# yardenas/ethz-safe-learning

Hardware: AMD Instinct MI355X
Metric: planning steps/sec (CEM-MPC, N=2000 K=5 H=30) (higher is better)
Workload: dtype f32

## Files before the change

ethz_safe_learning_amd/_capi.py:

```python
from __future__ import annotations

import ctypes as C
import os

CEM_ABI_VERSION = 4
CEM_MAX_ACT = 32
CEM_MAX_COST_KINDS = 4
CEM_COMM_ID_BYTES = 128
CEM_MAX_BATCH = 256
CEM_TRAIN_MAX_BATCH = 4096
CEM_INIT_COLD, CEM_INIT_EXPLICIT, CEM_INIT_SHIFT = 0, 1, 2
CEM_VARIANT_CEM, CEM_VARIANT_SAFE, CEM_VARIANT_COST = 0, 1, 2
CEM_PARTICLES_MEAN, CEM_PARTICLES_LOWER_TAIL = 0, 1
CEM_CONSTRAINT_BETA, CEM_CONSTRAINT_BUDGET = 0, 1
CEM_REFIT_UNIFORM, CEM_REFIT_SOFTMAX = 0, 1
CEM_FORWARD_SPLIT, CEM_FORWARD_ALL = 0, 1

_HERE = os.path.dirname(os.path.abspath(__file__))
LIB_PATH = os.environ.get('CEM_MPC_LIB') or os.path.join(_HERE, 'lib', 'libcem_mpc_gfx950.so')

EXPORTED_SYMBOLS = [
    'cem_abi_version', 'cem_status_string', 'cem_last_hip_error', 'cem_weight_blob_floats',
    'cem_packed_weight_floats', 'cem_workspace_bytes', 'cem_pack_weights_host', 'cem_plan_tiles_host', 'cem_plan_segments_host', 'cem_rollout_residency',
    'cem_planner_create', 'cem_planner_destroy', 'cem_planner_layout', 'cem_planner_set_weights', 'cem_planner_set_weights_dev',
    'cem_planner_set_normaliser', 'cem_planner_plan', 'cem_plan_begin', 'cem_plan_rollout', 'cem_plan_select',
    'cem_plan_end', 'cem_comm_unique_id', 'cem_planner_comm_init', 'cem_planner_comm_destroy', 'cem_planner_comm_ranks', 'cem_plan_exchange', 'cem_planner_graph_status', 'cem_planner_launches_per_iteration', 'cem_unfold_sequences', 'cem_compute_objective', 'cem_scorer_reward', 'cem_scorer_cost', 'cem_fill_noise', 'cem_philox_words', 'cem_planner_set_timing', 'cem_planner_last_timing', 'cem_planner_last_timing_detail', 'cem_planner_select_mode', 'cem_planner_inject_fault',
    'cem_batch_workspace_bytes', 'cem_batch_planner_create', 'cem_planner_plan_batch', 'cem_planner_batch_capacity',
    'cem_planner_set_warm_start', 'cem_planner_set_initial_distribution', 'cem_planner_set_init_mode', 'cem_planner_reset_carry',
    'cem_planner_get_carry', 'cem_planner_set_carry_slots', 'cem_planner_set_particle_objective', 'cem_planner_get_particle_objective',
    'cem_planner_set_constraint', 'cem_planner_get_constraint', 'cem_planner_set_cost_budget', 'cem_planner_constraint_costs',
    'cem_planner_set_refit', 'cem_planner_get_refit', 'cem_planner_refit_stats',
    'cem_trainer_workspace_bytes', 'cem_trainer_blob_floats', 'cem_trainer_create', 'cem_trainer_destroy', 'cem_trainer_set_state',
    'cem_trainer_get_state', 'cem_trainer_weights_dev', 'cem_trainer_step', 'cem_trainer_steps', 'cem_trainer_eval', 'cem_trainer_forward',
]


class CemScorer(C.Structure):
    _fields_ = [
        ('goal_mode', C.c_int32), ('goal_lo', C.c_int32), ('goal_hi', C.c_int32),
        ('lidar_max_dist', C.c_float), ('goal_size', C.c_float), ('goal_reached_dist', C.c_float), ('reward_distance', C.c_float),
        ('reward_goal', C.c_float), ('reward_clip', C.c_float),
        ('constrain_indicator', C.c_int32), ('n_cost_kinds', C.c_int32),
        ('cost_lo', C.c_int32 * CEM_MAX_COST_KINDS), ('cost_hi', C.c_int32 * CEM_MAX_COST_KINDS),
        ('cost_size', C.c_float * CEM_MAX_COST_KINDS),
    ]


class CemConfig(C.Structure):
    _fields_ = [
# ... 61 lines not shown
    lib.cem_pack_weights_host.argtypes = [cfgp, vp, vp]
    lib.cem_plan_tiles_host.argtypes = [cfgp, i32p, i32p, vp, C.c_int32]
    lib.cem_plan_segments_host.argtypes = [cfgp, i32p, i32p]
    lib.cem_rollout_residency.argtypes = [C.c_int32, C.c_int32, i32p, i32p]
    lib.cem_planner_create.argtypes = [cfgp, vp, C.c_size_t, vp, C.POINTER(vp)]
    lib.cem_planner_destroy.argtypes = [vp]
    lib.cem_planner_layout.argtypes = [vp, C.POINTER(CemLayout)]
    lib.cem_planner_set_weights.argtypes = [vp, vp, C.c_size_t]
    lib.cem_planner_set_weights_dev.argtypes = [vp, vp, C.c_size_t]
    lib.cem_planner_set_normaliser.argtypes = [vp, vp, vp]
    lib.cem_planner_plan.argtypes = [vp, vp, C.c_uint64, C.c_uint64, vp, vp, vp, vp, fp, i32p]
    lib.cem_plan_begin.argtypes = [vp, vp, C.c_uint64, C.c_uint64, vp, vp]
    lib.cem_plan_rollout.argtypes = [vp, C.c_int32]
    lib.cem_plan_select.argtypes = [vp, C.c_int32]
    lib.cem_plan_end.argtypes = [vp, vp, vp, fp, i32p]
    lib.cem_unfold_sequences.argtypes = [vp, vp, vp, C.c_int32, C.c_int32, vp, C.c_uint64, C.c_uint64, vp, vp, vp]
    lib.cem_comm_unique_id.argtypes = [vp]
    lib.cem_planner_comm_init.argtypes = [vp, vp, C.c_int32, C.c_int32]
    lib.cem_planner_comm_destroy.argtypes = [vp]
    lib.cem_plan_exchange.argtypes = [vp]
    lib.cem_planner_graph_status.argtypes = [vp, i32p]
    lib.cem_planner_comm_ranks.argtypes = [vp, i32p]
    lib.cem_planner_launches_per_iteration.argtypes = [vp, i32p]
    lib.cem_compute_objective.argtypes = [vp, vp, C.c_int32, C.c_int32, vp]
    lib.cem_scorer_reward.argtypes = [vp, vp, vp, C.c_int32, vp, vp]
    lib.cem_scorer_cost.argtypes = [vp, vp, C.c_int32, vp]
    lib.cem_fill_noise.argtypes = [vp, C.c_uint64, C.c_uint64, vp, vp, vp]
    lib.cem_philox_words.argtypes = [vp, C.c_uint64, C.c_uint64] + [C.c_uint32] * 6 + [vp]
    lib.cem_planner_select_mode.argtypes = [vp, i32p]
    lib.cem_planner_inject_fault.argtypes = [vp, C.c_int32]
    lib.cem_planner_set_timing.argtypes = [vp, C.c_int32]
    lib.cem_planner_last_timing.argtypes = [vp, fp, i32p, fp]
    lib.cem_planner_last_timing_detail.argtypes = [vp, fp, fp]
    lib.cem_batch_workspace_bytes.restype = C.c_size_t
    lib.cem_batch_workspace_bytes.argtypes = [cfgp, C.c_int32]
    lib.cem_batch_planner_create.argtypes = [cfgp, C.c_int32, vp, C.c_size_t, vp, C.POINTER(vp)]
    lib.cem_planner_plan_batch.argtypes = [vp, C.c_int32, vp, C.c_uint64, vp, vp, vp, vp, vp, vp, vp]
    lib.cem_planner_batch_capacity.argtypes = [vp, i32p]
    lib.cem_planner_set_warm_start.argtypes = [vp, C.POINTER(CemWarmStart)]
    lib.cem_planner_set_initial_distribution.argtypes = [vp, C.c_int32, vp, vp]
    lib.cem_planner_set_init_mode.argtypes = [vp, C.c_int32, C.c_int32]
    lib.cem_planner_reset_carry.argtypes = [vp, C.c_int32]
    lib.cem_planner_get_carry.argtypes = [vp, C.c_int32, vp, vp, i32p]
    lib.cem_planner_set_carry_slots.argtypes = [vp, C.c_int32, vp]
    lib.cem_planner_set_particle_objective.argtypes = [vp, C.c_int32, C.c_int32]
    lib.cem_planner_get_particle_objective.argtypes = [vp, i32p, i32p]
# ... 35 lines not shown
```

ethz_safe_learning_amd/csrc/cem_capi.hip:

```cpp
#include "cem_device.h"
#include "cem_score.h"
#include "cem_refit_weighted.h"
#include "cem_train.h"
#include "cem_train_tile.h"
#include "cem_forward.h"
#include "cem_rollout_split.h"
#include "cem_rollout_wide.h"
#include "cem_pack.h"
#include "../../include/cem_mpc.h"

#include <dlfcn.h>
#include <link.h>

#include <algorithm>
#include <atomic>
#include <chrono>
#include <cmath>
#include <cstdio>
#include <cstdlib>
#include <cstring>
#include <limits>
#include <mutex>
#include <new>
#include <string>
// ... 560 lines not shown
        dl_iterate_phdr(count_hip_runtimes, &libs);
        if (libs.size() > 1) {
            std::fprintf(stderr, "cem_mpc: %zu HIP runtimes are loaded in this process:", libs.size());
            for (const auto &l : libs) std::fprintf(stderr, " %s", l.c_str());
            std::fprintf(stderr, "\ncem_mpc: device memory and streams of one are foreign to the other — load libcem_mpc_gfx950.so AFTER the runtime that owns them (INTEGRATION.md)\n");
        }
    });
}
}

struct cem_planner {
    cem_config_t cfg;
    Dims d;
    Layout lay;
    char *ws;
    hipStream_t stream;
    bool own_stream;
    int rc;
    int n_tiles;
    int n_seg, seg_len, n_pinned;
    bool have_weights;
    bool in_plan;
    bool sample_in_rollout;
    const float *eps_act, *eps_model;
    CtrlBlock *h_ctrl;
    float *h_result;
    WarmCtl *h_warm; const WarmCtl *d_h_warm;
    uint32_t plan_seq;
    const CtrlBlock *d_h_ctrl; float *d_h_result;
    bool timing; std::vector<hipEvent_t> ev; float roll_ms, sel_ms, red_ms, samp_ms; int roll_n;
    std::vector<std::pair<int, int>> ev_kind;
    hipGraph_t graph; hipGraphExec_t gexec; bool graph_ready;
    ScorerDev sc;
    ScorerDev sc_roll;
    float alpha, beta;
    void *comm;
    int plans_since_comm;
    bool graph_failed;
    size_t sel_dyn_limit;
    int fused_resident;
    bool sel_zeroed;
    bool fuse_banned;
    bool inject_capture_fail;
    uint32_t inject_next;
    char *scratch; size_t scratch_bytes;
    std::vector<float> h_etab;
// ... 135 lines not shown
int cem_plan_segments_host(const cem_config_t *cfg, int32_t *segments_out, int32_t *steps_per_segment_out)
{
    int st = validate(cfg); if (st) return st;
    const Dims d = make_dims(cfg);
    const Plan pl = make_plan(cfg, d);
    if (segments_out) *segments_out = pl.n_seg;
    if (steps_per_segment_out) *steps_per_segment_out = pl.seg_len;
    return CEM_OK;
}

int cem_rollout_residency(int32_t chunks_per_tile, int32_t input_blocks_per_wave, int32_t *table_out, int32_t *runtime_out)
{
    if (chunks_per_tile < 1 || chunks_per_tile > 4 || input_blocks_per_wave < 1 || input_blocks_per_wave > 2) return CEM_ERR_INVALID_ARG;
    for (int seg = 0; seg < 2; ++seg) {
        if (table_out) table_out[seg] = kResidentStatic[seg][input_blocks_per_wave - 1][chunks_per_tile - 1];
        if (runtime_out)
            runtime_out[seg] = with_tile_shape(chunks_per_tile, input_blocks_per_wave, 0, [&](auto R, auto F) { return query_resident<R(), F()>(seg != 0); });
    }
    return CEM_OK;
}

}

static int planner_create(const cem_config_t *cfg, int32_t mb, void *workspace, size_t workspace_bytes, void *hip_stream, cem_planner_t **out)
{
    int st = mb ? validate_batch(cfg, mb) : validate(cfg); if (st) return st;
    if (!workspace || !out) return CEM_ERR_INVALID_ARG;
    warn_if_two_hip_runtimes();
    cem_planner *h = new (std::nothrow) cem_planner();
    if (!h) return CEM_ERR_INVALID_ARG;
    h->cfg = *cfg; h->d = make_dims(cfg);
    h->batch = mb; h->n_states = warm_slots(h);
    const size_t nb = (size_t)warm_slots(h);
    h->lay = make_layout(cfg, h->d, max_tiles_of(h->d), mb);
    if (workspace_bytes < h->lay.total || ((uintptr_t)workspace & 255)) { delete h; return CEM_ERR_WORKSPACE; }
    h->ws = (char *)workspace; h->stream = (hipStream_t)hip_stream; h->own_stream = false;
    if (!h->stream) {
        if (hipStreamCreateWithFlags(&h->stream, hipStreamNonBlocking) != hipSuccess) { g_last_hip = (int)hipGetLastError(); delete h; return CEM_ERR_HIP; }
        h->own_stream = true;
    }
    { const Plan pl = make_plan(cfg, h->d, mb); h->rc = pl.rc; h->n_seg = pl.n_seg; h->seg_len = pl.seg_len; h->n_pinned = pl.n_pinned;
      const int slots = real_cus() * ((h->d.wide || h->d.split) ? 1 : resident_workgroups(h->d.NFW, pl.rc, pl.n_seg > 1));
      h->sample_in_rollout = (long long)nb * pl.n_tiles <= slots;
      if (const char *e = std::getenv("CEM_FORCE_SAMPLER"))
          h->sample_in_rollout = std::strcmp(e, "kernel") != 0; }
    h->have_weights = false; h->in_plan = false; h->eps_act = h->eps_model = nullptr;
    h->timing = false; h->roll_ms = h->sel_ms = h->red_ms = h->samp_ms = 0.f; h->roll_n = 0;
    h->graph = nullptr; h->gexec = nullptr; h->graph_ready = false; h->tail_m = 0;
    h->cost_m = 0; h->budget_dev = nullptr; h->cstat_obj = nullptr; h->cstat_obj_n = 0; h->last_cstat = nullptr; h->last_cstat_n = h->last_cstat_problems = 0;
    h->refit_kind = CEM_REFIT_UNIFORM; h->refit_tau = 0.f; h->refit_beta = 0.f; h->refit_dev = nullptr; h->refit_ran = false;
    h->h_budget.assign(nb, std::numeric_limits<float>::infinity());
    h->comm = nullptr; h->plans_since_comm = 0; h->graph_failed = false;
    h->h_ctrl = nullptr; h->h_result = nullptr; h->h_warm = nullptr; h->d_h_warm = nullptr; h->pack_desc = nullptr; h->n_pack_desc = 0;
    h->warm = cem_warm_start_t{}; h->warm.shift = 1; h->warm_staged = 0; h->warm_save_skipped = false;
    h->slot_mode.assign(nb, CEM_INIT_COLD); h->carry_valid.assign(nb, 0); h->have_expl.assign(nb, 0); h->carry_at.assign(nb, -1);
    h->slot_of.resize(nb); for (size_t b = 0; b < nb; ++b) h->slot_of[b] = (int32_t)b;
    h->h_expl.assign(nb * 2 * h->d.H * h->d.A, 0.f);
    h->scratch = nullptr; h->scratch_bytes = 0; h->sel_zeroed = false; h->plan_seq = 0; h->fuse_banned = false; h->inject_next = 0; h->inject_capture_fail = false;
    auto fail = [&](int status) { g_last_hip = (int)hipGetLastError(); release_handle(h); return status; };
    const size_t result_bytes = mb ? nb * CEM_RESULT_WORDS * 4 : 64 * 4;
    if (hipHostMalloc((void **)&h->h_ctrl, nb * sizeof(CtrlBlock), hipHostMallocMapped | hipHostMallocCoherent) != hipSuccess ||
        hipHostMalloc((void **)&h->h_result, result_bytes, hipHostMallocMapped | hipHostMallocCoherent) != hipSuccess ||
        hipHostMalloc((void **)&h->h_warm, sizeof(WarmCtl) + nb * sizeof(WarmProb), hipHostMallocMapped | hipHostMallocCoherent) != hipSuccess) return fail(CEM_ERR_HIP);
    {
        const std::vector<PackDesc> table = build_pack_table(h->d);
        h->n_pack_desc = (uint32_t)table.size();
        const size_t image_bytes = h->d.wide ? wide_image_floats(h->d) * 4 : (size_t)h->d.member_stride_f4 * 16 - 4096;
        if (table.size() * (h->d.split ? 3072 : 1024) != image_bytes) return fail(CEM_ERR_STATE);
// ... 389 lines not shown
    const Dims &d = h->d; const Layout &l = h->lay; char *ws = h->ws;
    const bool queued = h->n_seg > 1 && !h->eps_model;
    RolloutParams rp; fill_rollout_common(h, rp);
    rp.tiles = (const TileDesc *)(ws + l.tiles); rp.s0 = nullptr; rp.actions = (const float *)(ws + l.actions);
    rp.eps_model = h->eps_model ? h->eps_model + (size_t)it * d.H * d.Btot * d.O : nullptr;
    const bool cost_obj = h->cfg.variant == CEM_VARIANT_COST;
    rp.ret = (float *)(ws + l.returns); rp.costs = h->cfg.variant != CEM_VARIANT_CEM ? (uint8_t *)(ws + l.costs) : nullptr;
    rp.H = d.H; rp.Bloc = d.Bloc; rp.Btot = d.Btot; rp.it = it; rp.variant = cost_obj ? (int)CEM_VARIANT_SAFE : h->cfg.variant; rp.check_done = 1;
    rp.stamps = (long long *)(ws + l.stamps);
    rp.musig = (const float *)(ws + l.musig); rp.eps_act = h->eps_act ? h->eps_act + (size_t)it * d.N * d.H * d.A : nullptr;
    rp.act_bounds = (const float *)(ws + l.act_bounds); rp.actions_w = (float *)(ws + l.actions); rp.act_pad_w = (float *)(ws + l.act_pad);
    rp.pad_shift = d.O - 4 * d.act_q0; rp.pad_floats = 4 * d.act_nq; rp.N = d.N; rp.Nloc = d.Nloc; rp.n_off = d.n_off; rp.n_tiles = h->n_tiles;
    const int nb = warm_slots(h);
    rp.tiles_per_problem = h->batch ? h->n_tiles : 0;
    rp.eps_act_pstride = (long long)d.I * d.N * d.H * d.A; rp.eps_model_pstride = (long long)d.I * d.H * d.Btot * d.O;
    if (!h->sample_in_rollout) {
        const int total = d.N * d.H * ((d.A + 3) / 4);
        TimedLaunch timed(h, 3);
        hipLaunchKernelGGL(cem_sample_kernel, dim3(std::min((total + 255) / 256, 2048), nb), dim3(256), 0, h->stream, rp);
        HIPCHK(hipGetLastError());
        rp.musig = nullptr;
    }
    TimedLaunch timed(h, 0);
    if (d.wide) HIPCHK(launch_rollout_wide(h, rp, h->n_tiles, rp.eps_model ? 1 : 0));
    else if (d.split) HIPCHK(launch_rollout_split(h->rc, d.NFW, rp.eps_model ? 1 : 0, rp, h->n_tiles, h->stream));
    else if (rp.eps_model) HIPCHK(launch_rollout<1>(h->rc, d.NFW, rp, nb * h->n_tiles, h->stream));
    else if (queued) {
        rp.seg_queue = (uint32_t *)(ws + l.seg_queue); rp.seg_flags = (uint32_t *)(ws + l.seg_flags); rp.seg_state = (f4 *)(ws + l.seg_state);
        rp.seg_len = h->seg_len; rp.n_seg = h->n_seg; rp.n_pinned = h->n_pinned;
        HIPCHK(launch_rollout_seg(h->rc, d.NFW, rp, h->n_pinned + h->n_seg * (h->n_tiles - h->n_pinned), h->stream));
    } else HIPCHK(launch_rollout<0>(h->rc, d.NFW, rp, nb * h->n_tiles, h->stream));
    timed.stop();
    if (fold_reduce) return CEM_OK;

    const ReduceParams sp = fill_score(h, rp.ret, rp.costs, (float *)(ws + l.scores_local), h->cost_m ? h->budget_dev + nb : nullptr, d.Nloc, d.H, 1, true);
    h->sel_zeroed = true;
    if (h->cost_m) note_plan_cstat(h);
    TimedLaunch timed_reduce(h, 2);
    HIPCHK(launch_score(h, sp, nb));
    return CEM_OK;
}

bool folds_reduce(const cem_planner *h)
{
    const Dims &d = h->d;
    if (d.W != 1 || h->comm || h->cfg.variant != CEM_VARIANT_CEM) return false;
    if (h->tail_m) return false;
// ... 635 lines not shown
    return CEM_OK;
}

int cem_planner_comm_destroy(cem_planner_t *h)
{
    if (!h) return CEM_ERR_INVALID_ARG;
    if (h->in_plan) return CEM_ERR_STATE;
    if (h->comm) {
        HIPCHK(hipStreamSynchronize(h->stream));
        if (Rccl *r = rccl()) r->CommDestroy(h->comm);
        h->comm = nullptr;
        drop_graph(h);
    }
    return CEM_OK;
}

int cem_planner_graph_status(const cem_planner_t *h, int32_t *status_out)
{
    if (!h || !status_out) return CEM_ERR_INVALID_ARG;
    *status_out = h->graph_ready ? 1 : (h->graph_failed ? 2 : 0);
    return CEM_OK;
}

int cem_planner_launches_per_iteration(const cem_planner_t *h, int32_t *launches_out)
{
    if (!h || !launches_out) return CEM_ERR_INVALID_ARG;
    const int mode = select_mode_now(h);
    *launches_out = 1 + (h->sample_in_rollout ? 0 : 1) + (folds_reduce(h) ? 0 : 1) + (mode == 2 ? 8 : (mode == 3 ? 2 : 1)) +
                    (h->refit_kind == CEM_REFIT_SOFTMAX ? 1 : 0);
    return CEM_OK;
}

int cem_plan_exchange(cem_planner_t *h)
{
    if (!h) return CEM_ERR_INVALID_ARG;
    if (!h->in_plan || !h->comm) return CEM_ERR_STATE;
    return enqueue_exchange(h);
}

static int ensure_scratch(cem_planner *h, size_t bytes)
{
    if (bytes <= h->scratch_bytes) return CEM_OK;
    if (h->scratch) { HIPCHK(hipStreamSynchronize(h->stream)); HIPCHK(hipFree(h->scratch)); h->scratch = nullptr; h->scratch_bytes = 0; }
    const size_t want = align256(bytes + bytes / 2);
    HIPCHK(hipMalloc((void **)&h->scratch, want));
    h->scratch_bytes = want;
// ... 459 lines not shown
```

ethz_safe_learning_amd/csrc/cem_device.h:

```cpp
#pragma once
#include <hip/hip_runtime.h>
#include <stdint.h>

typedef float f4 __attribute__((ext_vector_type(4)));

#define CEM_U 128
#define CEM_ET_NMIN 0
#define CEM_ET_RDELTA 1
#define CEM_ET_BMU 2
#define CEM_ET_BVAR 3
#define CEM_ET_OBS 4
#define CEM_ET_ACT 5
#define CEM_ET_SEL0 6
#define CEM_ET_SEL1 7
#define CEM_ET_ROWS 8
#define CEM_NG 8
#define CEM_NKIND 5
#define CEM_PART_FLOATS (CEM_NKIND * 4 * 64)
#define CEM_TAB_LDS_BYTES (CEM_ET_ROWS * CEM_U * 4)
#define CEM_ROLLOUT_LDS_BYTES(RC_) ((size_t)2 * (RC_) * CEM_NG * 1024 + CEM_PART_FLOATS * 4 + CEM_TAB_LDS_BYTES)

struct TileDesc {
    int32_t row_base;
    int32_t cnt;
// ... 361 lines not shown
    if (!p.musig) return;
    const TileDesc td = p.tiles[tile_idx];
    const bool natural = natural_all || td.row_base < p.Nloc;
    const int AZ = (p.A + 3) >> 2, nst = t1 - t0;
    const PhiloxKey key = cem_key(p.ctrl + b);
    const int own = td.cnt * nst * AZ;
    for (int idx = (int)threadIdx.x; idx < own; idx += 256) {
        const int z = idx % AZ, tt = (idx / AZ) % nst, r_ = idx / (AZ * nst);
        cem_sample_store(p, td.act_base + r_, t0 + tt, z, key, true, natural, b);
    }
    if (foreign && p.Nloc < p.N) {
        const long long total = (long long)(p.N - p.Nloc) * p.H * AZ;
        const long long per = (total + p.n_tiles - 1) / p.n_tiles;
        const long long lo = per * tile_idx, hi = (lo + per < total) ? lo + per : total;
        for (long long idx = lo + (long long)threadIdx.x; idx < hi; idx += 256) {
            const int z = (int)(idx % AZ), t = (int)((idx / AZ) % p.H);
            const int jn = (int)(idx / ((long long)AZ * p.H));
            cem_sample_store(p, jn < p.n_off ? jn : jn + p.Nloc, t, z, key, false);
        }
    }
    if (WAIT) cem_tile_sample_join();
}

__global__ __launch_bounds__(256) void cem_sample_kernel(const RolloutParams p)
{
    const int b = (int)blockIdx.y;
    if (p.check_done && p.ctrl[b].done) return;
    const int AZ = (p.A + 3) >> 2;
    const int total = p.N * p.H * AZ;
    const PhiloxKey key = cem_key(p.ctrl + b);
    for (int idx = blockIdx.x * blockDim.x + threadIdx.x; idx < total; idx += gridDim.x * blockDim.x) {
        const int z = idx % AZ, t = (idx / AZ) % p.H, n = idx / (AZ * p.H);
        cem_sample_store(p, n, t, z, key, true, true, b);
    }
}

#include "cem_rollout_common.h"

#define CEM_TAB(TABL_, ROW_, TV_) (*reinterpret_cast<const f4 *>((TABL_) + (ROW_) * 512 + (TV_)))
#define CEM_SEL0_LDS(TABL_, TV_) CEM_TAB(TABL_, CEM_ET_SEL0, TV_)

template <int RC, int NFW, int MODE, bool SEG>
__device__ __forceinline__ void cem_rollout_tile(const RolloutParams &p, char *smem, const int tile_idx, const int t_begin, const int t_end, const int b = 0)
{
    const int tid = (int)((threadIdx.x + 64u * (unsigned)((tile_idx + (tile_idx >> 8)) & 3)) & 255u);
    const int w = __builtin_amdgcn_readfirstlane(tid >> 6);
    const int lane = tid & 63;
    const int j = lane & 15, q = lane >> 4;
    const TileDesc td = p.tiles[tile_idx];
    const bool resumed = SEG && t_begin > 0;
    const int wbk = 0;
    const __amdgpu_buffer_rsrc_t seg_rs = __builtin_amdgcn_make_buffer_rsrc(
        SEG ? const_cast<f4 *>(p.seg_state + (size_t)(tile_idx - p.n_pinned) * (2 * NFW * RC * 256 + 64)) : const_cast<f4 *>(p.wpack), 0,
        (2 * NFW * RC * 256 + 64) * 16, 0x00020000);
    const int O = p.O, A = p.A, H = p.H;
    constexpr int XB = RC * CEM_NG * 1024;
    constexpr int LA = CEM_LDS_AHEAD_OF(RC, NFW);
    float *part = reinterpret_cast<float *>(smem + 2 * XB);
// ... 297 lines not shown
    const int tile = (int)(item >> 8), seg = (int)(item & 255u);
    const int t0 = seg * p.seg_len, t1 = (t0 + p.seg_len < p.H) ? t0 + p.seg_len : p.H;
    cem_tile_sample_actions<false>(p, tile, t0, t1 < p.H ? t1 + 1 : p.H, seg == 0, false);
    cem_rollout_tile<RC, NFW, 0, true>(p, smem, tile, t0, t1);
    if (t1 == p.H) {
        if (threadIdx.x == 0) item_s = atomicAdd(p.seg_queue + 2, 1u);
        __syncthreads();
        if (item_s == n_float - 1u) {
            const int n_ready = (int)n_float * (p.n_seg - 1);
            for (int i = (int)threadIdx.x; i < n_ready; i += 256) __hip_atomic_store(p.seg_flags + i, 0u, __ATOMIC_RELAXED, __HIP_MEMORY_SCOPE_AGENT);
            if (threadIdx.x < 3) __hip_atomic_store(p.seg_queue + threadIdx.x, 0u, __ATOMIC_RELAXED, __HIP_MEMORY_SCOPE_AGENT);
        }
    }
    if (t1 < p.H) {
        __builtin_amdgcn_s_waitcnt(0x0F70);
        __syncthreads();
        if (threadIdx.x == 0) {
            const uint32_t pos = atomicAdd(p.seg_queue + 1, 1u);
            __hip_atomic_store(p.seg_flags + pos, (((uint32_t)tile << 8) | (uint32_t)(seg + 1)) + 1u, __ATOMIC_RELAXED, __HIP_MEMORY_SCOPE_AGENT);
        }
    }
}

struct WarmProb {
    int32_t mode;
    int32_t slot;
    int32_t save_slot;
    int32_t pad;
};
struct WarmCtl { int32_t shift, tail, sigma_rule, two_phase ; float sigma_floor[32]; WarmProb prob[1];  };
#define CEM_WARM_LDS_PROBS 256

struct InitParams { CtrlBlock *ctrl; const CtrlBlock *host_ctrl; float *musig; int32_t HA, A; float mu0[32], sigma0[32]; uint32_t *seg_queue, *seg_flags; int32_t n_ready;
                    int32_t n_prob;
                    const WarmCtl *warm;
                    float *carry;
                    const float *expl;      };

__global__ void cem_init_kernel(const InitParams p)
{
    const int i = blockIdx.x * blockDim.x + threadIdx.x;
    const int np = p.n_prob > 1 ? p.n_prob : 1;
    WarmProb wp0{}; float fl0 = 0.f; int32_t hd0 = 0;
    if (blockIdx.x == 0) {
        if ((int)threadIdx.x < np) wp0 = p.warm->prob[threadIdx.x];
        if (threadIdx.x < 32) fl0 = p.warm->sigma_floor[threadIdx.x];
// ... 1186 lines not shown
    if (p.eps_act) {
        const int AZ = (p.A + 3) >> 2;
        const size_t total = (size_t)p.I * p.N * p.H * AZ;
        for (size_t idx = gid; idx < total; idx += gsz) {
            const int z = idx % AZ, t = (idx / AZ) % p.H, n = (idx / ((size_t)AZ * p.H)) % p.N, it = idx / ((size_t)AZ * p.H * p.N);
            const f4 e = cem_normal4((uint32_t)n, (uint32_t)t, (uint32_t)it, (uint32_t)z, CEM_STREAM_ACT, cem_key(p.ctrl));
            for (int r = 0; r < 4; ++r) if (4 * z + r < p.A) p.eps_act[(((size_t)it * p.N + n) * p.H + t) * p.A + 4 * z + r] = e[r];
        }
    }
    if (p.eps_model) {
        const int OZ = (p.O + 3) >> 2;
        const size_t total = (size_t)p.I * p.H * p.B * OZ;
        for (size_t idx = gid; idx < total; idx += gsz) {
            const int fq = idx % OZ; const size_t row = (idx / OZ) % p.B; const int t = (idx / ((size_t)OZ * p.B)) % p.H, it = idx / ((size_t)OZ * p.B * p.H);
            const f4 e = cem_normal4((uint32_t)row, (uint32_t)t, (uint32_t)it, (uint32_t)fq, CEM_STREAM_MODEL, cem_key(p.ctrl));
            for (int r = 0; r < 4; ++r) if (4 * fq + r < p.O) p.eps_model[(((size_t)it * p.H + t) * p.B + row) * p.O + 4 * fq + r] = e[r];
        }
    }
    if (p.eps_out && gid < (size_t)p.A) {
        const f4 e = cem_normal4((uint32_t)(gid >> 2), 0u, 0u, 0u, CEM_STREAM_OUT, cem_key(p.ctrl));
        p.eps_out[gid] = e[gid & 3];
    }
}
```

ethz_safe_learning_amd/planner.py:

```python
from __future__ import annotations

import ctypes as C
import math
from dataclasses import dataclass, field
from typing import List, Optional, Sequence, Tuple

import numpy as np

from . import _capi


@dataclass
class ScorerConfig:
    goal_slice: Tuple[int, int]
    observe_goal_lidar: bool = True
    lidar_max_dist: float = 4.0
    goal_size: float = 0.3
    reward_distance: float = 1.0
    reward_goal: float = 1.0
    reward_clip: float = 10.0
    constrain_indicator: bool = True
    cost_kinds: List[Tuple[int, int, float]] = field(default_factory=list)


# ... 320 lines not shown
        with self._torch.cuda.device(self.device):
            _capi.check(self.lib.cem_planner_comm_init(self.h, buf, c.world_size, c.rank), 'cem_planner_comm_init')
        self.has_comm = True

    def comm_ranks(self):
        n = C.c_int32()
        _capi.check(self.lib.cem_planner_comm_ranks(self.h, C.byref(n)), 'cem_planner_comm_ranks')
        return n.value

    def comm_destroy(self):
        _capi.check(self.lib.cem_planner_comm_destroy(self.h), 'cem_planner_comm_destroy')
        self.has_comm = False

    def graph_status(self):
        st = C.c_int32()
        _capi.check(self.lib.cem_planner_graph_status(self.h, C.byref(st)), 'cem_planner_graph_status')
        return ('eager', 'graph', 'graph-unsupported')[st.value]

    def launches_per_iteration(self):
        n = C.c_int32()
        _capi.check(self.lib.cem_planner_launches_per_iteration(self.h, C.byref(n)), 'cem_planner_launches_per_iteration')
        return n.value

    def set_particle_objective(self, kind='mean', m=0):
        if kind not in PARTICLE_OBJECTIVES:
            raise ValueError("kind is 'mean' or 'lower_tail'")
        _capi.check(self.lib.cem_planner_set_particle_objective(self.h, PARTICLE_OBJECTIVES[kind], int(m)), 'cem_planner_set_particle_objective')

    def particle_objective(self):
        kind, m = C.c_int32(), C.c_int32()
        _capi.check(self.lib.cem_planner_get_particle_objective(self.h, C.byref(kind), C.byref(m)), 'cem_planner_get_particle_objective')
        return ('mean', 'lower_tail')[kind.value], m.value

    def set_constraint(self, kind='beta', worst_cost_particles=0):
        if kind not in CONSTRAINTS:
            raise ValueError("kind is 'beta' or 'budget'")
        _capi.check(self.lib.cem_planner_set_constraint(self.h, CONSTRAINTS[kind], int(worst_cost_particles)), 'cem_planner_set_constraint')

    def constraint(self):
        kind, m = C.c_int32(), C.c_int32()
        _capi.check(self.lib.cem_planner_get_constraint(self.h, C.byref(kind), C.byref(m)), 'cem_planner_get_constraint')
        return ('beta', 'budget')[kind.value], m.value

    def set_cost_budget(self, budget):
        b = np.ascontiguousarray(np.asarray(budget, np.float32).reshape(-1))
        self.budget_staged = None
# ... 424 lines not shown
```

include/cem_mpc.h:

```cpp
#ifndef CEM_MPC_H
#define CEM_MPC_H

#include <stddef.h>
#include <stdint.h>

#ifdef __cplusplus
extern "C" {
#endif

#define CEM_ABI_VERSION 4
#define CEM_MAX_ACT 32
#define CEM_MAX_COST_KINDS 4
#define CEM_MAX_BATCH 256

enum cem_status {
    CEM_OK = 0,
    CEM_ERR_INVALID_ARG = 1,
    CEM_ERR_UNSUPPORTED = 2,
    CEM_ERR_SPLIT = 3,
    CEM_ERR_WORKSPACE = 4,
    CEM_ERR_HIP = 5,
    CEM_ERR_NO_WEIGHTS = 6,
    CEM_ERR_STATE = 7,
    CEM_ERR_COMM = 8,
// ... 94 lines not shown
int cem_planner_set_normaliser(cem_planner_t *h, const float *inputs_min, const float *inputs_max );
int cem_planner_set_weights_dev(cem_planner_t *h, const float *blob_dev, size_t n_floats);

int cem_planner_plan(cem_planner_t *h, const float *state, uint64_t seed, uint64_t call,
                     const float *eps_act_dev, const float *eps_model_dev, const float *eps_out_host,
                     float *action_out, float *best_score_out, int32_t *iters_out);

int cem_plan_begin(cem_planner_t *h, const float *state, uint64_t seed, uint64_t call,
                   const float *eps_act_dev, const float *eps_model_dev);
int cem_plan_rollout(cem_planner_t *h, int32_t it);
int cem_plan_select(cem_planner_t *h, int32_t it);
int cem_plan_end(cem_planner_t *h, const float *eps_out_host, float *action_out, float *best_score_out, int32_t *iters_out);

#define CEM_COMM_ID_BYTES 128
int cem_comm_unique_id(void *id_out );
int cem_planner_comm_init(cem_planner_t *h, const void *id , int32_t n_ranks, int32_t rank);
int cem_planner_comm_destroy(cem_planner_t *h);
int cem_planner_comm_ranks(const cem_planner_t *h, int32_t *n_ranks_out);
int cem_plan_exchange(cem_planner_t *h);
int cem_planner_select_mode(const cem_planner_t *h, int32_t *mode_out);
int cem_planner_inject_fault(cem_planner_t *h, int32_t kind);
int cem_planner_graph_status(const cem_planner_t *h, int32_t *status_out);
int cem_planner_launches_per_iteration(const cem_planner_t *h, int32_t *launches_out);

int cem_unfold_sequences(cem_planner_t *h, const float *s0_dev, const float *actions_dev, int32_t n_rows, int32_t horizon,
                         const float *eps_model_dev, uint64_t seed, uint64_t call,
                         float *traj_out_dev, float *mu_out_dev, float *sd_out_dev);

int cem_compute_objective(cem_planner_t *h, const float *traj_dev, int32_t n_rows, int32_t horizon, float *scores_out_dev);

int cem_scorer_reward(cem_planner_t *h, const float *obs_dev, const float *next_obs_dev, int32_t n, float *reward_out_dev,
                      uint8_t *goal_achieved_out_dev);
int cem_scorer_cost(cem_planner_t *h, const float *obs_dev, int32_t n, float *cost_out_dev);

int cem_fill_noise(cem_planner_t *h, uint64_t seed, uint64_t call, float *eps_act_dev, float *eps_model_dev, float *eps_out_dev);

int cem_philox_words(cem_planner_t *h, uint64_t seed, uint64_t call, uint32_t stream, uint32_t iteration, uint32_t t, uint32_t sub,
                     uint32_t idx0, uint32_t n, uint32_t *words_out_dev);

int cem_planner_set_timing(cem_planner_t *h, int32_t enable);
int cem_planner_last_timing(cem_planner_t *h, float *rollout_ms_total, int32_t *rollout_launches, float *select_ms_total);
int cem_planner_last_timing_detail(cem_planner_t *h, float *reduce_ms_total, float *sampler_ms_total);

size_t cem_batch_workspace_bytes(const cem_config_t *cfg, int32_t max_batch);
int cem_batch_planner_create(const cem_config_t *cfg, int32_t max_batch, void *workspace, size_t workspace_bytes, void *hip_stream,
                             cem_planner_t **out);
// ... 78 lines not shown
```

Baseline: 528.9.

## Add specialized lean rollout kernel for single-member, four-layer, RC=1 configurations

Adds a dedicated rollout kernel specialized for RC=1, NFW=1, four hidden layers and in-rollout sampling. It stages the action mean/sigma and bounds in LDS, computes clipped actions inline, and buffers kept actions in LDS so they are written out once at the end instead of per step. It also rotates wave priorities per step. The host picks this path automatically when eligible and keeps the generic path behind an environment override. The trade-off is extra LDS use and a second kernel to maintain. The weak symbol means the generic path is used if the new object is not linked.

```diff
diff --git a/ethz_safe_learning_amd/_capi.py b/ethz_safe_learning_amd/_capi.py
--- a/ethz_safe_learning_amd/_capi.py
+++ b/ethz_safe_learning_amd/_capi.py
@@ -24,7 +24,7 @@
     'cem_packed_weight_floats', 'cem_workspace_bytes', 'cem_pack_weights_host', 'cem_plan_tiles_host', 'cem_plan_segments_host', 'cem_rollout_residency',
     'cem_planner_create', 'cem_planner_destroy', 'cem_planner_layout', 'cem_planner_set_weights', 'cem_planner_set_weights_dev',
     'cem_planner_set_normaliser', 'cem_planner_plan', 'cem_plan_begin', 'cem_plan_rollout', 'cem_plan_select',
-    'cem_plan_end', 'cem_comm_unique_id', 'cem_planner_comm_init', 'cem_planner_comm_destroy', 'cem_planner_comm_ranks', 'cem_plan_exchange', 'cem_planner_graph_status', 'cem_planner_launches_per_iteration', 'cem_unfold_sequences', 'cem_compute_objective', 'cem_scorer_reward', 'cem_scorer_cost', 'cem_fill_noise', 'cem_philox_words', 'cem_planner_set_timing', 'cem_planner_last_timing', 'cem_planner_last_timing_detail', 'cem_planner_select_mode', 'cem_planner_inject_fault',
+    'cem_plan_end', 'cem_comm_unique_id', 'cem_planner_comm_init', 'cem_planner_comm_destroy', 'cem_planner_comm_ranks', 'cem_plan_exchange', 'cem_planner_graph_status', 'cem_planner_launches_per_iteration', 'cem_planner_rollout_path', 'cem_unfold_sequences', 'cem_compute_objective', 'cem_scorer_reward', 'cem_scorer_cost', 'cem_fill_noise', 'cem_philox_words', 'cem_planner_set_timing', 'cem_planner_last_timing', 'cem_planner_last_timing_detail', 'cem_planner_select_mode', 'cem_planner_inject_fault',
     'cem_batch_workspace_bytes', 'cem_batch_planner_create', 'cem_planner_plan_batch', 'cem_planner_batch_capacity',
     'cem_planner_set_warm_start', 'cem_planner_set_initial_distribution', 'cem_planner_set_init_mode', 'cem_planner_reset_carry',
     'cem_planner_get_carry', 'cem_planner_set_carry_slots', 'cem_planner_set_particle_objective', 'cem_planner_get_particle_objective',
@@ -132,6 +132,7 @@
     lib.cem_planner_graph_status.argtypes = [vp, i32p]
     lib.cem_planner_comm_ranks.argtypes = [vp, i32p]
     lib.cem_planner_launches_per_iteration.argtypes = [vp, i32p]
+    lib.cem_planner_rollout_path.argtypes = [vp, i32p]
     lib.cem_compute_objective.argtypes = [vp, vp, C.c_int32, C.c_int32, vp]
     lib.cem_scorer_reward.argtypes = [vp, vp, vp, C.c_int32, vp, vp]
     lib.cem_scorer_cost.argtypes = [vp, vp, C.c_int32, vp]
diff --git a/ethz_safe_learning_amd/csrc/cem_capi.hip b/ethz_safe_learning_amd/csrc/cem_capi.hip
--- a/ethz_safe_learning_amd/csrc/cem_capi.hip
+++ b/ethz_safe_learning_amd/csrc/cem_capi.hip
@@ -1,4 +1,5 @@
 #include "cem_device.h"
+#include "cem_rollout_lean.h"
 #include "cem_score.h"
 #include "cem_refit_weighted.h"
 #include "cem_train.h"
@@ -606,6 +607,7 @@
     bool have_weights;
     bool in_plan;
     bool sample_in_rollout;
+    bool lean_rollout;
     const float *eps_act, *eps_model;
     CtrlBlock *h_ctrl;
     float *h_result;
@@ -787,6 +789,13 @@
 
 }
 
+static bool lean_eligible(const cem_planner *h, int rc)
+{
+    const Dims &d = h->d;
+    return launch_rollout_lean != nullptr && !d.wide && !d.split && rc == 1 && d.NFW == 1 && d.L == 4 && d.O % 4 == 0 && h->cfg.world_size == 1 && !h->batch &&
+           h->sample_in_rollout && CEM_LEAN_ACT_LDS_BYTES(d.H, (d.A + 3) / 4) <= CEM_LEAN_ACT_LDS_MAX;
+}
+
 static int planner_create(const cem_config_t *cfg, int32_t mb, void *workspace, size_t workspace_bytes, void *hip_stream, cem_planner_t **out)
 {
     int st = mb ? validate_batch(cfg, mb) : validate(cfg); if (st) return st;
@@ -808,7 +817,10 @@
       const int slots = real_cus() * ((h->d.wide || h->d.split) ? 1 : resident_workgroups(h->d.NFW, pl.rc, pl.n_seg > 1));
       h->sample_in_rollout = (long long)nb * pl.n_tiles <= slots;
       if (const char *e = std::getenv("CEM_FORCE_SAMPLER"))
-          h->sample_in_rollout = std::strcmp(e, "kernel") != 0; }
+          h->sample_in_rollout = std::strcmp(e, "kernel") != 0;
+      h->lean_rollout = lean_eligible(h, pl.rc);
+      if (const char *e = std::getenv("CEM_FORCE_ROLLOUT"))
+          h->lean_rollout = h->lean_rollout && std::strcmp(e, "generic") != 0; }
     h->have_weights = false; h->in_plan = false; h->eps_act = h->eps_model = nullptr;
     h->timing = false; h->roll_ms = h->sel_ms = h->red_ms = h->samp_ms = 0.f; h->roll_n = 0;
     h->graph = nullptr; h->gexec = nullptr; h->graph_ready = false; h->tail_m = 0;
@@ -1244,7 +1256,14 @@
         rp.musig = nullptr;
     }
     TimedLaunch timed(h, 0);
-    if (d.wide) HIPCHK(launch_rollout_wide(h, rp, h->n_tiles, rp.eps_model ? 1 : 0));
+    if (h->lean_rollout && !rp.eps_act && !rp.eps_model) {
+        if (queued) {
+            rp.seg_queue = (uint32_t *)(ws + l.seg_queue); rp.seg_flags = (uint32_t *)(ws + l.seg_flags); rp.seg_state = (f4 *)(ws + l.seg_state);
+            rp.seg_len = h->seg_len; rp.n_seg = h->n_seg; rp.n_pinned = h->n_pinned;
+        }
+        HIPCHK(launch_rollout_lean(rp, queued ? h->n_pinned + h->n_seg * (h->n_tiles - h->n_pinned) : h->n_tiles, h->stream, queued));
+    }
+    else if (d.wide) HIPCHK(launch_rollout_wide(h, rp, h->n_tiles, rp.eps_model ? 1 : 0));
     else if (d.split) HIPCHK(launch_rollout_split(h->rc, d.NFW, rp.eps_model ? 1 : 0, rp, h->n_tiles, h->stream));
     else if (rp.eps_model) HIPCHK(launch_rollout<1>(h->rc, d.NFW, rp, nb * h->n_tiles, h->stream));
     else if (queued) {
@@ -1926,6 +1945,13 @@
     return CEM_OK;
 }
 
+int cem_planner_rollout_path(const cem_planner_t *h, int32_t *path_out)
+{
+    if (!h || !path_out) return CEM_ERR_INVALID_ARG;
+    *path_out = h->lean_rollout ? 1 : 0;
+    return CEM_OK;
+}
+
 int cem_planner_launches_per_iteration(const cem_planner_t *h, int32_t *launches_out)
 {
     if (!h || !launches_out) return CEM_ERR_INVALID_ARG;
diff --git a/ethz_safe_learning_amd/csrc/cem_device.h b/ethz_safe_learning_amd/csrc/cem_device.h
--- a/ethz_safe_learning_amd/csrc/cem_device.h
+++ b/ethz_safe_learning_amd/csrc/cem_device.h
@@ -407,6 +407,7 @@
     if (WAIT) cem_tile_sample_join();
 }
 
+#ifndef CEM_DEVICE_PRIMITIVES_ONLY
 __global__ __launch_bounds__(256) void cem_sample_kernel(const RolloutParams p)
 {
     const int b = (int)blockIdx.y;
@@ -419,6 +420,7 @@
         cem_sample_store(p, n, t, z, key, true, true, b);
     }
 }
+#endif
 
 #include "cem_rollout_common.h"
 
@@ -762,6 +764,7 @@
     }
 }
 
+#ifndef CEM_DEVICE_PRIMITIVES_ONLY
 struct WarmProb {
     int32_t mode;
     int32_t slot;
@@ -1994,3 +1997,4 @@
         p.eps_out[gid] = e[gid & 3];
     }
 }
+#endif
diff --git a/ethz_safe_learning_amd/csrc/cem_rollout_lean.h b/ethz_safe_learning_amd/csrc/cem_rollout_lean.h
--- /dev/null
+++ b/ethz_safe_learning_amd/csrc/cem_rollout_lean.h
@@ -0,0 +1,8 @@
+#pragma once
+#include "cem_device.h"
+
+#define CEM_LEAN_ACT_LDS_BYTES(H_, AZ_) (((size_t)(H_) + 1) * (AZ_) * (32 + 17 * 16))
+#define CEM_LEAN_LDS_BYTES(H_, AZ_) (CEM_ROLLOUT_LDS_BYTES(1) + CEM_LEAN_ACT_LDS_BYTES(H_, AZ_))
+#define CEM_LEAN_ACT_LDS_MAX 16384
+
+__attribute__((weak)) hipError_t launch_rollout_lean(const RolloutParams &p, int grid, hipStream_t st, bool seg);
diff --git a/ethz_safe_learning_amd/csrc/cem_rollout_lean.hip b/ethz_safe_learning_amd/csrc/cem_rollout_lean.hip
--- /dev/null
+++ b/ethz_safe_learning_amd/csrc/cem_rollout_lean.hip
@@ -0,0 +1,324 @@
+#define CEM_DEVICE_PRIMITIVES_ONLY
+#include "cem_rollout_lean.h"
+
+namespace {
+
+template <int V> struct LeanConst { static constexpr int value = V; };
+
+template <int KF, int NOWN, bool L0IN>
+__device__ __forceinline__ void cem_lean_stage(f4 (&acc0)[1], f4 (&acc1)[1], f4 (&hB)[CEM_NG][1], WRing &wq, const char *const *rb, const int xoff)
+{
+    static_assert(KF % 4 == 0, "stage lengths must keep the ring phase");
+#pragma unroll
+    for (int P = 0; P < KF; ++P) {
+        wq.slot[(P + 3) & 3] = wq.ld(wq.pos);
+        wq.pos = (wq.pos + 1 == wq.n) ? 0 : wq.pos + 1;
+        __builtin_amdgcn_sched_barrier(0);
+        if (P == 1) {
+            __syncthreads();
+#pragma unroll
+            for (int Q = NOWN; Q < KF; ++Q) hB[Q][0] = *reinterpret_cast<const f4 *>(rb[Q - NOWN] + xoff + (Q - NOWN) * 1024);
+        }
+        const AGroup g = wq.slot[P & 3];
+        const int Pb = (!L0IN && P < 2) ? (P ^ 1) : P;
+#pragma unroll
+        for (int r = 0; r < 4; ++r) {
+            acc0[0] = CEM_MFMA(g.a[r], hB[P][0][r], acc0[0]);
+            acc1[0] = CEM_MFMA(g.b[r], hB[Pb][0][r], acc1[0]);
+        }
+    }
+}
+
+template <bool SEG>
+__device__ __forceinline__ void cem_lean_tile(const RolloutParams &p, char *smem, const int tile_idx, const int t_begin, const int t_end)
+{
+    constexpr int RC = 1, NFW = 1;
+    const int tid = (int)((threadIdx.x + 64u * (unsigned)((tile_idx + (tile_idx >> 8)) & 3)) & 255u);
+    const int w = __builtin_amdgcn_readfirstlane(tid >> 6);
+    const int lane = tid & 63;
+    const int j = lane & 15, q = lane >> 4;
+    const TileDesc td = p.tiles[tile_idx];
+    const bool resumed = SEG && t_begin > 0;
+    const int wbk = 0;
+    const __amdgpu_buffer_rsrc_t seg_rs = __builtin_amdgcn_make_buffer_rsrc(
+        SEG ? const_cast<f4 *>(p.seg_state + (size_t)(tile_idx - p.n_pinned) * (2 * 256 + 64)) : const_cast<f4 *>(p.wpack), 0, (2 * 256 + 64) * 16, 0x00020000);
+    const int O = p.O, A = p.A, H = p.H, AZ = (A + 3) >> 2;
+    constexpr int XB = CEM_NG * 1024;
+    float *part = reinterpret_cast<float *>(smem + 2 * XB);
+    const CtrlBlock *const ctrl = p.ctrl;
+    const PhiloxKey key = cem_key(ctrl);
+    const float rscale = p.sampling ? CEM_BM_RSCALE : 0.0f;
+
+    const int member_u = __builtin_amdgcn_readfirstlane(td.member);
+    WRing wq;
+    wq.init(p.wpack + (size_t)member_u * p.member_stride_f4 + p.wave_off_f4[w], lane, (int)p.wave_groups[w]);
+
+    const __amdgpu_buffer_rsrc_t et_rs = __builtin_amdgcn_make_buffer_rsrc(
+        const_cast<float *>(p.etab + (size_t)member_u * (CEM_ET_ROWS + p.L) * CEM_U), 0, (CEM_ET_ROWS + p.L) * CEM_U * 4, 0x00020000);
+    const int tab_v = 64 * w + 16 * q;
+    const int bias_v = 128 * w + 16 * q;
+    const char *tabl = smem + 2 * XB + CEM_PART_FLOATS * 4;
+    const char *actl = tabl + CEM_TAB_LDS_BYTES;
+    {
+        const int ht = (int)threadIdx.x;
+        *reinterpret_cast<f4 *>(const_cast<char *>(tabl) + ht * 16) = cem_ld_tab(et_rs, (ht & 31) * 16, (ht >> 5) * 512);
+        const int HA = H * A;
+        for (int idx = ht; idx < (H + 1) * AZ; idx += 256) {
+            const int t = idx / AZ, z = idx - t * AZ;
+            const float *lo = t < H ? p.musig + HA + t * A : p.act_bounds, *hi = t < H ? p.musig + t * A : p.act_bounds + 32;
+            f4 u = {0.f, 0.f, 0.f, 0.f}, v = u;
+#pragma unroll
+            for (int r = 0; r < 4; ++r) if (4 * z + r < A) { u[r] = lo[4 * z + r]; v[r] = hi[4 * z + r]; }
+            *reinterpret_cast<f4 *>(const_cast<char *>(actl) + idx * 32) = u;
+            *reinterpret_cast<f4 *>(const_cast<char *>(actl) + idx * 32 + 16) = v;
+        }
+    }
+    __syncthreads();
+
+    f4 s[NFW][RC];
+    const int slot0 = j < td.cnt ? j : td.cnt - 1;
+    {
+        const int f0 = 16 * w + 4 * q;
+        if (resumed) s[0][0] = cem_ld_coherent(seg_rs, tid * 16);
+        else {
+#pragma unroll
+            for (int r = 0; r < 4; ++r) {
+                const int f = f0 + r;
+                float v = 0.f;
+                if (f < O) v = td.s0_base < 0 ? ctrl->state[f] : p.s0[(size_t)(td.s0_base + slot0) * O + f];
+                s[0][0][r] = v;
+            }
+        }
+    }
+
+    const int zq = 4 * w + q - (O >> 2);
+    const bool actlane = zq >= 0 && zq < AZ;
+    const bool wact = 4 * w + 3 >= (O >> 2) && 4 * w < (O >> 2) + AZ;
+    const int zc = actlane ? zq : 0;
+    const uint32_t pc0 = (uint32_t)((actlane ? td.act_base : td.noise_row_base) + slot0);
+    const uint32_t pc2 = actlane ? ((uint32_t)zc | (CEM_STREAM_ACT << 16)) : ((uint32_t)(4 * w + q) | (CEM_STREAM_MODEL << 16));
+    const uint32_t pc1 = ((uint32_t)p.it << 16) + (actlane ? 1u : 0u);
+    const float prs = actlane ? CEM_BM_RSCALE : rscale;
+    const char *const actl_v = actl + zc * 32;
+#define CEM_LEAN_ACTION(DST, E_, T_) do { \
+        const char *m_ = actl_v + (T_) * AZ * 32, *b_ = actl_v + H * AZ * 32; \
+        const f4 sg_ = *reinterpret_cast<const f4 *>(m_), mu_ = *reinterpret_cast<const f4 *>(m_ + 16); \
+        const f4 lb_ = *reinterpret_cast<const f4 *>(b_), ub_ = *reinterpret_cast<const f4 *>(b_ + 16); \
+        f4 v_ = (E_) * sg_; v_ = v_ + mu_; \
+        _Pragma("unroll") for (int r = 0; r < 4; ++r) DST[r] = fminf(fmaxf(v_[r], lb_[r]), ub_[r]); } while (0)
+    const bool act_keep = actlane && j < td.cnt && td.row_base < p.Nloc;
+    char *const stage = const_cast<char *>(actl) + (H + 1) * AZ * 32;
+    char *const stage_v = stage + ((act_keep ? j : 16) * (H + 1) * AZ + zc) * 16;
+#define CEM_LEAN_KEEP(V_, T_) do { *reinterpret_cast<f4 *>(stage_v + (T_) * AZ * 16) = (V_); } while (0)
+
+    float d_prev = 0.f, c_prev = 0.f, cum = 0.f;
+    bool done = false;
+    const int nk = 1 + p.sc.n_cost;
+    const float csz[4] = {p.sc.cost_size[0], p.sc.cost_size[1], p.sc.cost_size[2], p.sc.cost_size[3]};
+    const float ind_cap = p.sc.indicator ? 1.0f : __builtin_inff(), clipv = p.sc.reward_clip > 0.f ? p.sc.reward_clip : __builtin_inff();
+    const __amdgpu_buffer_rsrc_t cost_rs = __builtin_amdgcn_make_buffer_rsrc(p.costs, 0, p.costs ? (uint32_t)(H * p.Bloc) : 0u, 0x00020000);
+
+    f4 hB[CEM_NG][RC];
+    if (resumed) {
+        const f4 x = cem_ld_coherent(seg_rs, (256 + tid) * 16);
+        hB[0][0] = x;
+        *reinterpret_cast<f4 *>(smem + (w * 64 + lane) * 16) = x;
+        if (w == wbk) {
+            const f4 b = cem_ld_coherent(seg_rs, (2 * 256 + lane) * 16);
+            d_prev = b[0]; c_prev = b[1]; cum = b[2]; done = b[3] != 0.f;
+        }
+    } else {
+        float pm[2][RC];
+        pm[0][0] = __builtin_inff(); pm[1][0] = __builtin_inff();
+        const int tv = tab_v;
+        const f4 mn4 = CEM_TAB(tabl, CEM_ET_NMIN, tv), rd4 = CEM_TAB(tabl, CEM_ET_RDELTA, tv);
+        const f4 isact4 = CEM_TAB(tabl, CEM_ET_ACT, tv);
+        const f4 sel0 = CEM_TAB(tabl, CEM_ET_SEL0, tv), sel1 = CEM_TAB(tabl, CEM_ET_SEL1, tv);
+        const f4 e0 = cem_normal4(pc0, 0u, (uint32_t)p.it, (uint32_t)zc, CEM_STREAM_ACT, key);
+        const f4 sn = s[0][0];
+        f4 xin = sn;
+        if (wact) {
+            f4 act4; CEM_LEAN_ACTION(act4, e0, 0);
+            CEM_LEAN_KEEP(act4, 0);
+            xin = __builtin_elementwise_fma(isact4, act4, sn);
+        }
+        cem_scorer_terms(sn, p.sc.D, sel0, sel1, pm[0][0], pm[1][0]);
+        const f4 x = cem_sub4(xin, mn4) * rd4;
+        *reinterpret_cast<f4 *>(smem + (w * 64 + lane) * 16) = x;
+        hB[0][0] = x;
+        CEM_RARE_KINDS_AND_STORE(RC, NFW, p, part, w, q, j, nk, s, pm, tab_v, CEM_SEL0_LDS, tabl);
+    }
+    f4 nb0 = cem_ld_tab(et_rs, bias_v, CEM_ET_ROWS * 512);
+    f4 nb1 = cem_ld_tab(et_rs, bias_v + 64, CEM_ET_ROWS * 512);
+
+    const char *rbh[6], *rb0[3];
+#pragma unroll
+    for (int k = 0; k < 6; ++k) rbh[k] = smem + lane * 16 + (k < 2 * w ? 0 : 2048);
+#pragma unroll
+    for (int k = 0; k < 3; ++k) rb0[k] = smem + lane * 16 + (k < w ? 0 : 1024);
+    char *const pubh = smem + (2 * w * 64 + lane) * 16, *const pub0 = smem + (w * 64 + lane) * 16;
+    const bool prio_rot = !(SEG && tile_idx >= p.n_pinned);
+    const int prio_r0 = (tile_idx >> 8) % 3;
+    auto step = [&](auto XW0, const int t, const bool first) __attribute__((always_inline)) {
+        int xw = decltype(XW0)::value;
+        if (prio_rot) {
+            const int lvl = (t + prio_r0) % 3;
+            if (lvl == 0) __builtin_amdgcn_s_setprio(0); else if (lvl == 1) __builtin_amdgcn_s_setprio(1); else __builtin_amdgcn_s_setprio(2);
+        }
+#define CEM_RELU_PUBLISH() do { \
+            f4 h0 = acc0[0], h1 = acc1[0]; \
+            _Pragma("unroll") for (int r = 0; r < 4; ++r) { h0[r] = fmaxf(h0[r], 0.f); h1[r] = fmaxf(h1[r], 0.f); } \
+            *reinterpret_cast<f4 *>(pubh + xw) = h0; \
+            *reinterpret_cast<f4 *>(pubh + xw + 1024) = h1; \
+            hB[0][0] = h0; hB[1][0] = h1; \
+            xw ^= XB; } while (0)
+#define CEM_NEXT_BIAS(LN) do { \
+            nb0 = cem_ld_tab(et_rs, bias_v, (CEM_ET_ROWS + (LN)) * 512); \
+            nb1 = cem_ld_tab(et_rs, bias_v + 64, (CEM_ET_ROWS + (LN)) * 512); } while (0)
+        {
+            f4 acc0[RC], acc1[RC];
+            acc0[0] = nb0; acc1[0] = nb1;
+            CEM_NEXT_BIAS(1);
+            cem_lean_stage<4, 1, true>(acc0, acc1, hB, wq, rb0, xw ^ XB);
+            if (!(resumed && first)) CEM_BOOKKEEP(p, td, part, w, wbk, lane, nk, csz, ind_cap, clipv, cost_rs, d_prev, c_prev, cum, done, t - 1);
+            CEM_RELU_PUBLISH();
+        }
+#pragma unroll
+        for (int l = 1; l < 4; ++l) {
+            f4 acc0[RC], acc1[RC];
+            acc0[0] = nb0; acc1[0] = nb1;
+            CEM_NEXT_BIAS(l + 1 < 4 ? l + 1 : 0);
+            cem_lean_stage<CEM_NG, 2, false>(acc0, acc1, hB, wq, rbh, xw ^ XB);
+            CEM_RELU_PUBLISH();
+        }
+#undef CEM_RELU_PUBLISH
+#undef CEM_NEXT_BIAS
+
+        float pm[2][RC];
+        pm[0][0] = __builtin_inff(); pm[1][0] = __builtin_inff();
+        const int tn = (t + 1 < H) ? t + 1 : H - 1;
+        {
+            const int Fo = w;
+            const int tv = tab_v;
+            f4 accm[RC], accv[RC];
+            accm[0] = CEM_TAB(tabl, CEM_ET_BMU, tv); accv[0] = CEM_TAB(tabl, CEM_ET_BVAR, tv);
+            if (Fo < p.KB_obs) cem_lean_stage<CEM_NG, 2, false>(accm, accv, hB, wq, rbh, xw ^ XB);
+            else __syncthreads();
+            const f4 e4 = cem_normal4(pc0, pc1 + (uint32_t)t, 0u, pc2, 0u, key, prs);
+            const f4 mn4 = CEM_TAB(tabl, CEM_ET_NMIN, tv), rd4 = CEM_TAB(tabl, CEM_ET_RDELTA, tv);
+            const f4 om4 = CEM_TAB(tabl, CEM_ET_OBS, tv), isact4 = CEM_TAB(tabl, CEM_ET_ACT, tv);
+            const f4 sel0 = CEM_TAB(tabl, CEM_ET_SEL0, tv), sel1 = CEM_TAB(tabl, CEM_ET_SEL1, tv);
+
+            const f4 mu = accm[0];
+            const f4 var = cem_softplus4(accv[0]) + 1e-4f;
+            f4 sd;
+#pragma unroll
+            for (int r = 0; r < 4; ++r) sd[r] = __builtin_amdgcn_sqrtf(var[r]);
+            const f4 d = mu + sd * e4;
+            const f4 sn = s[0][0] + d * om4;
+            s[0][0] = sn;
+            cem_scorer_terms(sn, p.sc.D, sel0, sel1, pm[0][0], pm[1][0]);
+            f4 xin = sn;
+            if (wact) {
+                f4 act4; CEM_LEAN_ACTION(act4, e4, tn);
+                CEM_LEAN_KEEP(act4, t + 1);
+                xin = __builtin_elementwise_fma(isact4, act4, sn);
+            }
+            const f4 x = cem_sub4(xin, mn4) * rd4;
+            *reinterpret_cast<f4 *>(pub0 + xw) = x;
+            hB[0][0] = x;
+        }
+        CEM_RARE_KINDS_AND_STORE(RC, NFW, p, part, w, q, j, nk, s, pm, tab_v, CEM_SEL0_LDS, tabl);
+    };
+    for (int t = t_begin; t < t_end; t += 2) {
+        step(LeanConst<XB>{}, t, t == t_begin);
+        if (t + 1 >= t_end) break;
+        step(LeanConst<0>{}, t + 1, false);
+    }
+#undef CEM_LEAN_ACTION
+#undef CEM_LEAN_KEEP
+    __syncthreads();
+    CEM_BOOKKEEP(p, td, part, w, wbk, lane, nk, csz, ind_cap, clipv, cost_rs, d_prev, c_prev, cum, done, t_end - 1);
+    if (td.row_base < p.Nloc) {
+        const int tlo = resumed ? t_begin + 1 : 0, thi = t_end < H ? t_end : H - 1;
+        const int per = (thi - tlo + 1) * A;
+        const float *const stagef = reinterpret_cast<const float *>(stage);
+        for (int idx = (int)threadIdx.x; idx < td.cnt * per; idx += 256) {
+            const int row = idx / per, rem = idx - row * per, tt = tlo + rem / A, a = rem - (rem / A) * A;
+            p.actions_w[((size_t)(td.act_base + row) * H + tt) * A + a] = stagef[((row * (H + 1) + tt) * AZ) * 4 + a];
+        }
+    }
+    if (!SEG || t_end == H) {
+        if (w == wbk && lane < td.cnt) p.ret[td.row_base + lane] = cum;
+    } else {
+        cem_st_coherent(seg_rs, tid * 16, s[0][0]);
+        cem_st_coherent(seg_rs, (256 + tid) * 16, hB[0][0]);
+        if (w == wbk) cem_st_coherent(seg_rs, (2 * 256 + lane) * 16, (f4){d_prev, c_prev, cum, done ? 1.0f : 0.0f});
+    }
+}
+
+}
+
+__global__ __launch_bounds__(256) void cem_rollout_lean_kernel(const RolloutParams p)
+{
+    extern __shared__ __attribute__((aligned(16))) char smem[];
+    if (p.check_done && p.ctrl->done) return;
+    cem_lean_tile<false>(p, smem, (int)blockIdx.x, 0, p.H);
+}
+
+__global__ __launch_bounds__(256) void cem_rollout_lean_seg_kernel(const RolloutParams p)
+{
+    extern __shared__ __attribute__((aligned(16))) char smem[];
+    __shared__ uint32_t item_s;
+    if (p.check_done && p.ctrl->done) return;
+    if ((int)blockIdx.x < p.n_pinned) {
+        cem_lean_tile<true>(p, smem, (int)blockIdx.x, 0, p.H);
+        return;
+    }
+    __builtin_amdgcn_s_setprio(CEM_FLOAT_PRIO);
+    const uint32_t n_float = (uint32_t)(p.n_tiles - p.n_pinned);
+    if (threadIdx.x == 0) {
+        const uint32_t ticket = atomicAdd(p.seg_queue, 1u);
+        uint32_t item = (((uint32_t)p.n_pinned + ticket) << 8);
+        if (ticket >= n_float) {
+            const uint32_t *slot = p.seg_flags + (ticket - n_float);
+            uint32_t spins = 0, v;
+            while ((v = __hip_atomic_load(slot, __ATOMIC_RELAXED, __HIP_MEMORY_SCOPE_AGENT)) == 0u && ++spins < CEM_SEG_SPIN_LIMIT)
+                __builtin_amdgcn_s_sleep(16);
+            item = v ? v - 1u : 0xffffffffu;
+            if (!v) atomicOr(const_cast<int32_t *>(&p.ctrl->fault), 1 );
+        }
+        item_s = item;
+    }
+    __syncthreads();
+    const uint32_t item = item_s;
+    if (item == 0xffffffffu) return;
+    const int tile = (int)(item >> 8), seg = (int)(item & 255u);
+    const int t0 = seg * p.seg_len, t1 = (t0 + p.seg_len < p.H) ? t0 + p.seg_len : p.H;
+    cem_lean_tile<true>(p, smem, tile, t0, t1);
+    if (t1 == p.H) {
+        if (threadIdx.x == 0) item_s = atomicAdd(p.seg_queue + 2, 1u);
+        __syncthreads();
+        if (item_s == n_float - 1u) {
+            const int n_ready = (int)n_float * (p.n_seg - 1);
+            for (int i = (int)threadIdx.x; i < n_ready; i += 256) __hip_atomic_store(p.seg_flags + i, 0u, __ATOMIC_RELAXED, __HIP_MEMORY_SCOPE_AGENT);
+            if (threadIdx.x < 3) __hip_atomic_store(p.seg_queue + threadIdx.x, 0u, __ATOMIC_RELAXED, __HIP_MEMORY_SCOPE_AGENT);
+        }
+    }
+    if (t1 < p.H) {
+        __builtin_amdgcn_s_waitcnt(0x0F70);
+        __syncthreads();
+        if (threadIdx.x == 0) {
+            const uint32_t pos = atomicAdd(p.seg_queue + 1, 1u);
+            __hip_atomic_store(p.seg_flags + pos, (((uint32_t)tile << 8) | (uint32_t)(seg + 1)) + 1u, __ATOMIC_RELAXED, __HIP_MEMORY_SCOPE_AGENT);
+        }
+    }
+}
+
+hipError_t launch_rollout_lean(const RolloutParams &p, int grid, hipStream_t st, bool seg)
+{
+    const size_t lds = CEM_LEAN_LDS_BYTES(p.H, (p.A + 3) / 4);
+    if (seg) hipLaunchKernelGGL(cem_rollout_lean_seg_kernel, dim3(grid), dim3(256), lds, st, p);
+    else hipLaunchKernelGGL(cem_rollout_lean_kernel, dim3(grid), dim3(256), lds, st, p);
+    return hipGetLastError();
+}
diff --git a/ethz_safe_learning_amd/planner.py b/ethz_safe_learning_amd/planner.py
--- a/ethz_safe_learning_amd/planner.py
+++ b/ethz_safe_learning_amd/planner.py
@@ -366,6 +366,11 @@
         _capi.check(self.lib.cem_planner_launches_per_iteration(self.h, C.byref(n)), 'cem_planner_launches_per_iteration')
         return n.value
 
+    def rollout_path(self):
+        n = C.c_int32()
+        _capi.check(self.lib.cem_planner_rollout_path(self.h, C.byref(n)), 'cem_planner_rollout_path')
+        return ('generic', 'lean')[n.value]
+
     def set_particle_objective(self, kind='mean', m=0):
         if kind not in PARTICLE_OBJECTIVES:
             raise ValueError("kind is 'mean' or 'lower_tail'")
diff --git a/include/cem_mpc.h b/include/cem_mpc.h
--- a/include/cem_mpc.h
+++ b/include/cem_mpc.h
@@ -140,6 +140,7 @@
 int cem_planner_inject_fault(cem_planner_t *h, int32_t kind);
 int cem_planner_graph_status(const cem_planner_t *h, int32_t *status_out);
 int cem_planner_launches_per_iteration(const cem_planner_t *h, int32_t *launches_out);
+int cem_planner_rollout_path(const cem_planner_t *h, int32_t *path_out);
 
 int cem_unfold_sequences(cem_planner_t *h, const float *s0_dev, const float *actions_dev, int32_t n_rows, int32_t horizon,
                          const float *eps_model_dev, uint64_t seed, uint64_t call,
```

After: 542.6 (median of 6 runs). +2.6%, better.
